# cisco/openh264

Hardware: AMD Instinct MI355X
Metric: 1080p frames/sec/GPU at QP=24 CBP; encoder_binary_comparison SHA1 pass (higher is better)
Workload: dtype u8

## Files before the change

openh264_amd/csrc/kernels/inter_mb.h:

```cpp
#pragma once
#include "frame_kernels.h"
#include "../common/gom_rc.h"


#if defined(WH_EMU)
#include <stdio.h>
static long g_wh_win_stat[40];
static void wh_win_stat_dump() {
  if (!getenv ("WELSHIP_WIN_STATS")) return;
  fprintf (stderr, "welship mb stat: skip %ld bg/static %ld intra %ld p16x16 %ld p16x8 %ld p8x16 %ld p8x8 %ld renamed-skip %ld | searches 16x16 %ld 16x8/8x16 %ld 8x8 %ld, diamond steps %ld %ld %ld | refinements %ld %ld %ld | skip tests %ld with transform %ld\n",
           g_wh_win_stat[8], g_wh_win_stat[9], g_wh_win_stat[10], g_wh_win_stat[11], g_wh_win_stat[12], g_wh_win_stat[13], g_wh_win_stat[14], g_wh_win_stat[15], g_wh_win_stat[16], g_wh_win_stat[17], g_wh_win_stat[18],
           g_wh_win_stat[19], g_wh_win_stat[20], g_wh_win_stat[21], g_wh_win_stat[22], g_wh_win_stat[23], g_wh_win_stat[24], g_wh_win_stat[25], g_wh_win_stat[26]);
  fprintf (stderr, "welship window stat: P macroblocks %ld, reloads %ld, adopted %ld, first loads %ld, mid-walk reloads %ld, chroma predictions inside the window %ld / from the picture %ld\n", g_wh_win_stat[0], g_wh_win_stat[1], g_wh_win_stat[2], g_wh_win_stat[3], g_wh_win_stat[4], g_wh_win_stat[5], g_wh_win_stat[6]);
}
struct WhWinStatInit { WhWinStatInit() { atexit (wh_win_stat_dump); } };
static WhWinStatInit g_wh_win_stat_init;
#define WH_STAT_WIN(i) (++g_wh_win_stat[i])
#define WH_STAT_BLK(base, bw, bh) (++g_wh_win_stat[(base) + ((bw) == 16 && (bh) == 16 ? 0 : (bw) == 8 && (bh) == 8 ? 2 : 1)])
#else
#define WH_STAT_WIN(i) ((void)0)
#define WH_STAT_BLK(base, bw, bh) ((void)0)
#endif

#define WH_REF_NOT_AVAIL (-2)
#define WH_REF_NOT_IN_LIST (-1)
#define WH_WIN_STRIDE 80
#ifndef WH_WIN_ROWS
#define WH_WIN_ROWS 38
#endif
#define WH_WIN_MARGIN_X 19
#ifndef WH_WIN_MARGIN_Y
#define WH_WIN_MARGIN_Y 11
#endif
#ifndef WH_WIN_START
#define WH_WIN_START 5
#endif
#define WH_CWIN_STRIDE 64
#ifndef WH_CWIN_ROWS
#define WH_CWIN_ROWS 24
#endif
#define WH_CWIN_COLS 32

#define WH_SLOT_16x16 0
#define WH_SLOT_8x8 1
#define WH_SLOT_16x8 5
#define WH_SLOT_8x16 7

typedef struct alignas (16) WhWinLds {
  alignas (16) uint8_t win[WH_WIN_ROWS * WH_WIN_STRIDE + 16];
  alignas (16) uint8_t cwin[WH_CWIN_ROWS * WH_CWIN_STRIDE + 16];
} WhWinLds;

typedef struct alignas (16) WhInterLds {
  WhMbLds m;
  uint32_t nb[5 * 36];
  int16_t co_mv[2][2];
  uint32_t sad_cost0_in;
  int16_t mvp_out[16][2];
  int16_t mv_out[16][2];
} WhInterLds;

typedef struct alignas (16) WhInterStage {
  uint32_t cold_pv[64];
} WhInterStage;
typedef struct WhWin { int x0, y0, cx0, cy0; WhWinLds* b; } WhWin;

WH_FN int wh_se_bits (int v) {
// ... 619 lines not shown
#define WH_RF_ACT (lane < nq && (!sub8 || (bw == 16 ? ((lane >> 2) & 3) < 2 : lane < 16)))
#define WH_RF_ENC wh_enc4 (S, ex + (lane < nq ? wh_tl_col (lane, bw) : 0), ey + (lane < nq ? wh_tl_row (lane, bw) : 0))
#define WH_RF_O (wo + (lane < nq ? wh_tl_row (lane, bw) * WH_WIN_STRIDE + wh_tl_col (lane, bw) : 0))
  const int dmx = me.mvx - me.mvpx, dmy = me.mvy - me.mvpy;
  WvLaneArr vG, vhu, vhd, vbl, vbr, vq0, vq1, vq2, vq3;
#if defined(WH_EMU)
  memset (&vG, 0, sizeof (vG)); memset (&vhu, 0, sizeof (vhu)); memset (&vhd, 0, sizeof (vhd)); memset (&vbl, 0, sizeof (vbl)); memset (&vbr, 0, sizeof (vbr));
  memset (&vq0, 0, sizeof (vq0)); memset (&vq1, 0, sizeof (vq1)); memset (&vq2, 0, sizeof (vq2)); memset (&vq3, 0, sizeof (vq3));
#else
  vG = 0; vhu = 0; vhd = 0; vbl = 0; vbr = 0; vq0 = 0; vq1 = 0; vq2 = 0; vq3 = 0;
#endif
  int c_int, c0, c1, c2, c3;
  WV_DECLARE_LANE (lane);
  WV_LANE_EVAL (lane, {
    const int o = WH_RF_O;
    uint32_t a, b;
    WV_LOWN (vG, lane) = (int)wh_ld4u (W.b->win, o);
    wh_rf_h_pair (W.b->win, o, &a, &b); WV_LOWN (vhu, lane) = (int)a; WV_LOWN (vhd, lane) = (int)b;
    wh_rf_b_pair (W.b->win, o, &a, &b); WV_LOWN (vbl, lane) = (int)a; WV_LOWN (vbr, lane) = (int)b; });
  if (satd_in_md) c_int = me.satd_raw;
  else WV_SATD_ROWS_SHARED (c_int, lane, WH_RF_ACT, WH_RF_ENC, (uint32_t)WV_LOWN (vG, lane));
  WV_SATD_ROWS4_SHARED (c0, c1, c2, c3, lane, WH_RF_ACT, WH_RF_ENC, (uint32_t)WV_LOWN (vhu, lane), (uint32_t)WV_LOWN (vhd, lane), (uint32_t)WV_LOWN (vbl, lane), (uint32_t)WV_LOWN (vbr, lane));
  int best = c_int + wh_mvd_cost (C.lambda, dmx, dmy), hb = -1;
  c0 += wh_mvd_cost (C.lambda, dmx, dmy - 2); if (c0 < best) { best = c0; hb = 0; }
  c1 += wh_mvd_cost (C.lambda, dmx, dmy + 2); if (c1 < best) { best = c1; hb = 1; }
  c2 += wh_mvd_cost (C.lambda, dmx - 2, dmy); if (c2 < best) { best = c2; hb = 2; }
  c3 += wh_mvd_cost (C.lambda, dmx + 2, dmy); if (c3 < best) { best = c3; hb = 3; }
  const int hx = hb == 2 ? -2 : hb == 3 ? 2 : 0, hy = hb == 0 ? -2 : hb == 1 ? 2 : 0;
  WV_LANE_EVAL (lane, {
    uint32_t q[4];
    wh_rf_quarters (W.b->win, WH_RF_O, hb, (uint32_t)WV_LOWN (vG, lane), (uint32_t)WV_LOWN (vhu, lane), (uint32_t)WV_LOWN (vhd, lane), (uint32_t)WV_LOWN (vbl, lane), (uint32_t)WV_LOWN (vbr, lane), q);
    WV_LOWN (vq0, lane) = (int)q[0]; WV_LOWN (vq1, lane) = (int)q[1]; WV_LOWN (vq2, lane) = (int)q[2]; WV_LOWN (vq3, lane) = (int)q[3]; });
  WV_SATD_ROWS4_SHARED (c0, c1, c2, c3, lane, WH_RF_ACT, WH_RF_ENC, (uint32_t)WV_LOWN (vq0, lane), (uint32_t)WV_LOWN (vq1, lane), (uint32_t)WV_LOWN (vq2, lane), (uint32_t)WV_LOWN (vq3, lane));
  int qb = -1;
  c0 += wh_mvd_cost (C.lambda, dmx + hx, dmy + hy - 1); if (c0 < best) { best = c0; qb = 0; }
  c1 += wh_mvd_cost (C.lambda, dmx + hx, dmy + hy + 1); if (c1 < best) { best = c1; qb = 1; }
  c2 += wh_mvd_cost (C.lambda, dmx + hx - 1, dmy + hy); if (c2 < best) { best = c2; qb = 2; }
  c3 += wh_mvd_cost (C.lambda, dmx + hx + 1, dmy + hy); if (c3 < best) { best = c3; qb = 3; }
  const int qx = qb == 2 ? -1 : qb == 3 ? 1 : 0, qy = qb == 0 ? -1 : qb == 1 ? 1 : 0;
  me.satd_cost = best;
  WV_LANE_EVAL (lane, {
    if (lane < nq) {
      const int v = qb >= 0 ? (qb == 0 ? WV_LOWN (vq0, lane) : qb == 1 ? WV_LOWN (vq1, lane) : qb == 2 ? WV_LOWN (vq2, lane) : WV_LOWN (vq3, lane))
                  : hb >= 0 ? (hb == 0 ? WV_LOWN (vhu, lane) : hb == 1 ? WV_LOWN (vhd, lane) : hb == 2 ? WV_LOWN (vbl, lane) : WV_LOWN (vbr, lane)) : WV_LOWN (vG, lane);
      * (uint32_t*)&S.m.pred_y[(ey + wh_tl_row (lane, bw)) * 16 + ex + wh_tl_col (lane, bw)] = (uint32_t)v;
    } });
  WV_SYNC();
#undef WH_RF_ACT
#undef WH_RF_ENC
#undef WH_RF_O
  me.mvx += hx + qx; me.mvy += hy + qy;
}

WH_FN int wh_enc_inter_y (WhMbLds& S, int qp) {
  wh_quant_blocks (S, 0, 16, qp, qp, S.res, 0);
  int s0, s1, s2, s3;
  WV_QUADSUM4 (s0, s1, s2, s3, lane, (lane < 16 ? WH_Q_SCORE (S.part2[lane]) : 0));
  int cbp = 0;
  if (s0 + s1 + s2 + s3 >= 6) cbp = (s0 >= 4 ? 1 : 0) | (s1 >= 4 ? 2 : 0) | (s2 >= 4 ? 4 : 0) | (s3 >= 4 ? 8 : 0);
  WV_LANES_BEGIN (lane)
  {
    const int b = lane >> 2, on = (cbp >> (b >> 2)) & 1;
    for (int q = 0; q < 4; ++q) { const int k = (lane & 3) * 4 + q; S.lv_luma[b * 16 + k] = S.res[b * 16 + wh_zigzag (k)]; }
    if (lane < 16) {
      int n = 0;
      if ((cbp >> (lane >> 2)) & 1) n = __builtin_popcount (WH_Q_MASK (S.part2[lane]));
      S.nzc[wh_blk_y (lane) * 4 + wh_blk_x (lane)] = (uint8_t)n;
    }
    (void)on;
  }
  WV_LANES_END
  WV_LANES_BEGIN (lane)
  {
    const int b = lane >> 2, on = (cbp >> (b >> 2)) & 1;
    for (int k = 0; k < 4; ++k) {
      const int i = lane * 4 + k, pos = i & 15;
      S.res[i] = on ? (int16_t) (S.res[i] * wh_dq (qp, pos)) : (int16_t)0;
    }
  }
  WV_LANES_END
  return cbp;
}

WH_FN bool wh_try_py_skip (WhMbLds& S, int qp) {
  wh_quant_blocks (S, 0, 16, qp, qp, S.tmp, 0);
  int bc, u1, u2, u3;
  WV_ROWSUM4 (bc, u1, u2, u3, lane, (lane < 16 ? WH_Q_SCORE (S.part2[lane]) | (WH_Q_BIG (S.part2[lane]) << 16) : 0));
  (void)u1; (void)u2; (void)u3;
  return bc < 6;
}
WH_FN bool wh_try_puv_skip (WhMbLds& S, int qpc) {
  const int ff = wh_ff_inter (qpc, 0) << 1, mf = wh_mf (qpc, 0) >> 1;
  const int16_t thr = (int16_t) (((1 << 16) - 1) / mf - ff);
  for (int pl = 0; pl < 2; ++pl) {
    const int16_t* r = &S.res[256 + pl * 64];
    const int16_t s0 = (int16_t) (r[0] + r[32]), s1 = (int16_t) (r[0] - r[32]), s2 = (int16_t) (r[16] + r[48]), s3 = (int16_t) (r[16] - r[48]);
    const int16_t d0 = (int16_t) (s0 + s2), d1 = (int16_t) (s0 - s2), d2 = (int16_t) (s1 + s3), d3 = (int16_t) (s1 - s3);
    if (wh_abs (d0) > thr || wh_abs (d1) > thr || wh_abs (d2) > thr || wh_abs (d3) > thr) return false;
  }
  wh_quant_blocks (S, 256, 8, qpc, qpc, S.tmp, 1);
  int c0, c1, c2, c3;
  WV_QUADSUM4 (c0, c1, c2, c3, lane, (lane < 8 ? WH_Q_SCORE (S.part2[lane]) | (WH_Q_BIG (S.part2[lane]) << 8) : 0));
  (void)c2; (void)c3;
  return c0 < 7 && c1 < 7;
}

template <int VAR = 0>
WH_FN void wh_inter_cold_fetch (WhInterLds& S, WhInterStage& G, int lane, const WhSeqParams& P, const WhPicJob& J, int mbx, int mby) {
  constexpr bool HOSTIN = VAR == 0 || VAR == 3, CTRL = VAR == 0;
  const int w = P.mb_w, xy = mby * w + mbx;
  wh_ld_async4 ((const WH_G uint8_t*)J.src[0] + WH_SRC_Y_OFF (w, mbx, mby, 0, 0) + lane * 4, (uint32_t*)S.m.enc_y, lane);
  if (lane < 32) wh_ld_async4 ((const WH_G uint8_t*)J.src[0] + WH_SRC_C_OFF (w, mbx, mby, 0, 0, 0) + lane * 4, (uint32_t*)S.m.enc_c, lane);
// ... 120 lines not shown
  }
  const bool bg_cur = bgd && WV_LGET (bgf, 0) != 0, bg_l = bgd && WV_LGET (bgf, 1) != 0, bg_t = bgd && WV_LGET (bgf, 2) != 0;
  const bool bg_tr = bgd && WV_LGET (bgf, 3) != 0, bg_tl = bgd && WV_LGET (bgf, 4) != 0;
  const bool tl_skc = tl_sk && !bg_tl, t_skc = t_sk && !bg_t, tr_skc = tr_sk && !bg_tr, l_skc = l_sk && !bg_l;
  const int sadsk0 = tl_skc ? TLm->skip_sad : 0, sadsk1 = t_skc ? Tm->skip_sad : 0, sadsk2 = tr_skc ? TRm->skip_sad : 0, sadsk3 = l_skc ? Lm->skip_sad : 0;
  const int ref_mb_type = ref_is_p ? Co->mb_type : WH_MB_NONE;
  const bool ref_mb_bg = Co->ref_type == WH_REFTYPE_BACKGROUND;
  WhMeCtx C;
  C.mbx = mbx; C.mby = mby; C.lambda = lambda; C.use_satd = use_satd;
  C.minx = wh_max (- ((mbx + 1) << 4) + 3, -P.mv_range); C.miny = wh_max (- ((mby + 1) << 4) + 3, -P.mv_range);
  C.maxx = wh_min (((P.mb_w - mbx) << 4) - 3, P.mv_range); C.maxy = wh_min (((P.mb_h - mby) << 4) - 3, P.mv_range);

  WH_PROF_MARK (P, M, 10);
  WhMe me16;
  me16.bx = 0; me16.by = 0; me16.bw = 16; me16.bh = 16;
  wh_pred_mv (K, 0, 0, 4, 0, &me16.mvpx, &me16.mvpy);
  WhWin W;
  W.b = X.win;
  WhI16Cost i16c;
  {
    const int icx = wh_clip3 ((2 + me16.mvpx) >> 2, C.minx, C.maxx), icy = wh_clip3 ((2 + me16.mvpy) >> 2, C.miny, C.maxy);
    const int cx = mbx * 16 + icx, cy = mby * 16 + icy;
    const bool adopt = X.spec_valid && wh_win_room (X.spec, cx, cy, 16, 16) >= WH_WIN_START;
    WH_STAT_WIN (0);
    if (adopt) { W.x0 = X.spec.x0; W.y0 = X.spec.y0; W.cx0 = X.spec.cx0; W.cy0 = X.spec.cy0; WH_STAT_WIN (2); WH_PROF_MARK (P, M, 15); }
    else {
      WH_STAT_WIN (3);
      if (X.spec_valid) WV_ASYNC_WAIT();
      wh_win_issue_all (P, J, W, cx, cy);
    }
    wh_i16_costs (M, avail, use_satd, lambda, &i16c);
    WV_ASYNC_WAIT();
  }
  WH_PROF_MARK (P, M, 0);
  int mb_type = WH_MB_P16x16, cbp = 0, cost_luma = 0, cost_skip_mb = 0, sad_cost0 = 0;
  int p16x = 0, p16y = 0;
  int skx = 0, sky = 0;
  bool done = false;

  auto predict_sad_skip = [&] () {
    const int rb = WV_LGET (K.ref, 1), ra = WV_LGET (K.ref, 6);
    int rc = WV_LGET (K.ref, 5);
    const int sb = sadsk1, sa = sadsk3;
    int sc = sadsk2, skip_c = tr_skc;
    if (rc == WH_REF_NOT_AVAIL) { rc = WV_LGET (K.ref, 0); sc = sadsk0; skip_c = tl_skc; }
    if (rb == WH_REF_NOT_AVAIL && rc == WH_REF_NOT_AVAIL && ra != WH_REF_NOT_AVAIL) return sa;
    const int cnt = ((0 == ra) && l_skc) | (((0 == rb) && t_skc) << 1) | (((0 == rc) && skip_c) << 2);
    return cnt == 1 ? sa : cnt == 2 ? sb : cnt == 4 ? sc : wh_median3 (sa, sb, sc);
  };
  const bool try_skip = l_sk || t_sk || tl_sk || tr_sk;
  bool keep_skip = l_sk && t_sk && tr_sk;
  bool b_skip = false;
  const int stale_cbp = ctl.stale_cbp;
  bool bg_coded = false, bg_skip = false, collocated = false;

  if (bgd) {
    keep_skip = keep_skip && !bg_l && !bg_t && !bg_tr;
    const int ref_type_raw = (int)Co->ref_type - 1;
    const bool ref_intra = Co->ref_type != 0 && Co->ref_type != WH_REFTYPE_BACKGROUND && WH_IS_INTRA (ref_type_raw);
    const int ref_qp = Co->ref_qp;
    if (bg_cur && !ref_intra && (ref_qp - qp <= 3  || ref_qp <= 26)) {
      wh_mc_chroma_to (S, P, J, W, mbx, mby, 0, 0, 8, 8, 0, 0, M.pred_c);
      int cb, cr;
      WV_SUM2 (cb, cr, lane, (lane < 16 ? wh_sad4 (* (const uint32_t*)&M.enc_c[lane * 4], * (const uint32_t*)&M.pred_c[lane * 4]) : 0),
               (lane >= 16 && lane < 32 ? wh_sad4 (* (const uint32_t*)&M.enc_c[lane * 4], * (const uint32_t*)&M.pred_c[lane * 4]) : 0));
      const bool too_large = cb > 640 || cr > 640;
      const int chroma_sad = cb + cr, pred_skip = predict_sad_skip();
      const bool cannot = (pred_skip > 128 && chroma_sad >= pred_skip) ||
                          (ref_is_p && ref_mb_type == WH_MB_PSKIP && !ref_mb_bg && Co->skip_sad > 128 && chroma_sad >= Co->skip_sad);
      if (!cannot && !too_large) {
        int sx, sy;
        wh_pred_skip_mv (K, &sx, &sy);
        bg_coded = true; bg_skip = sx == 0 && sy == 0; collocated = true;
        wh_mc_luma_to (S, P, J, W, mbx, mby, 0, 0, 16, 16, 0, 0, M.pred_y);
        const uint8_t* pl = M.pred_y;
        int sad;
        WV_SUM (sad, lane, wh_sad4 (* (const uint32_t*)&M.enc_y[lane * 4], * (const uint32_t*)&pl[lane * 4]));
        sad_cost0 = sad;
        p16x = 0; p16y = 0;
        if (bg_skip) { b_skip = true; mb_type = WH_MB_PSKIP; skx = 0; sky = 0; cost_luma = 0; cost_skip_mb = 0; done = true; }
        else {
          mb_type = WH_MB_P16x16;
          if (md_using_sad) cost_luma = sad;
          else WV_SATD_ROWS (cost_luma, lane, true, wh_enc4 (S, wh_tl_col (lane, 16), wh_tl_row (lane, 16)), * (const uint32_t*)&M.pred_y[wh_tl_row (lane, 16) * 16 + wh_tl_col (lane, 16)]);
          WV_LANES_BEGIN (lane)
          if (lane < 16) { S.mv_out[lane][0] = 0; S.mv_out[lane][1] = 0; S.mvp_out[lane][0] = (int16_t)me16.mvpx; S.mvp_out[lane][1] = (int16_t)me16.mvpy; }
          WV_LANES_END
          wh_dct_luma16 (M);
          cbp = wh_enc_inter_y (M, qp);
          cbp |= wh_encrec_chroma (M, qpc, 0) << 4;
          wh_idct_luma16 (M);
          wh_idct_chroma (M);
          done = true;
        }
      }
    }
  }

  const WH_G WhSccJob* Z = nullptr;
  int idc0 = 0, idc1 = 0, idc2 = 0, idc3 = 0, scroll_on = 0, smx = 0, smy = 0;
  uint32_t dch0 = 0, dch1 = 0, dch2 = 0, dch3 = 0, fme_down_mb = 0;
  bool scd_coded = false;
  if (SCC) {
    Z = (const WH_G WhSccJob*)J.scc;
    const int scd_on = Z->scd_on;
    if (scd_on) {
// ... 23 lines not shown
        const WH_G uint8_t* o0 = (const WH_G uint8_t*)Z->ref_ori_c[0];
        const WH_G uint8_t* o1 = (const WH_G uint8_t*)Z->ref_ori_c[1];
        const ptrdiff_t off = (ptrdiff_t) ((mby << 3) + (oy >> 1)) * P.src_stride_c + (mbx << 3) + (ox >> 1);
        WV_SUM2 (cb, cr, lane,
                 (lane < 16 ? wh_sad4 (* (const uint32_t*)&M.enc_c[lane * 4], wh_ldg4u (o0 + off + (ptrdiff_t) ((lane >> 1) & 7) * P.src_stride_c + (lane & 1) * 4)) : 0),
                 (lane >= 16 && lane < 32 ? wh_sad4 (* (const uint32_t*)&M.enc_c[lane * 4], wh_ldg4u (o1 + off + (ptrdiff_t) ((lane >> 1) & 7) * P.src_stride_c + (lane & 1) * 4)) : 0));
      }
      if (cb != 0 || cr != 0) continue;
      const int ref_qp = Co->ref_qp;
      const bool qp_similar = ref_qp - qp <= 5  || ref_qp <= 26;
      int sx, sy;
      wh_pred_skip_mv (K, &sx, &sy);
      const int vx = (int) (int16_t) (ox * 4), vy = (int) (int16_t) (oy * 4);
      const bool as_skip = qp_similar && sx == vx && sy == vy;
      uint8_t* dy = M.pred_y;
      uint8_t* dc = M.pred_c;
      wh_mc_luma_to (S, P, J, W, mbx, mby, 0, 0, 16, 16, vx, vy, dy);
      wh_mc_chroma_to (S, P, J, W, mbx, mby, 0, 0, 8, 8, vx, vy, dc);
      int sad;
      WV_SUM (sad, lane, wh_sad4 (* (const uint32_t*)&M.enc_y[lane * 4], * (const uint32_t*)&dy[lane * 4]));
      sad_cost0 = sad; cost_skip_mb = sad;
      p16x = vx; p16y = vy;
      scd_coded = true;
      if (as_skip) { b_skip = true; mb_type = WH_MB_PSKIP; skx = vx; sky = vy; cost_luma = 0; collocated = vx == 0 && vy == 0; done = true; WH_STAT (mode ? WH_ST_SCROLL_SKIP : WH_ST_STATIC_SKIP); }
      else {
        WH_STAT (WH_ST_SCD_P16);
        mb_type = WH_MB_P16x16;
        collocated = false;
        if (md_using_sad) cost_luma = sad;
        else cost_luma = wh_cand_sad (S, P, J, W, C, me16, 0, 0);
        WV_LANES_BEGIN (lane)
        if (lane < 16) { S.mv_out[lane][0] = (int16_t)vx; S.mv_out[lane][1] = (int16_t)vy; S.mvp_out[lane][0] = (int16_t)me16.mvpx; S.mvp_out[lane][1] = (int16_t)me16.mvpy; }
        WV_LANES_END
        me16.mvx = vx; me16.mvy = vy;
        wh_dct_luma16 (M);
        cbp = wh_enc_inter_y (M, qp);
        cbp |= wh_encrec_chroma (M, qpc, 0) << 4;
        wh_idct_luma16 (M);
        wh_idct_chroma (M);
        done = true;
      }
    }
  }

  if (!done && ((ref_is_p && ref_mb_type == WH_MB_PSKIP) || try_skip)) {
    const int sad_pred_skip = predict_sad_skip();
    wh_pred_skip_mv (K, &skx, &sky);
    const int nx = (mbx << 4) + (skx >> 2), ny = (mby << 4) + (sky >> 2);
    if (!(nx < -29 || nx > (P.mb_w << 4) + 12 || ny < -29 || ny > (P.mb_h << 4) + 12)) {
      wh_mc_luma_to (S, P, J, W, mbx, mby, 0, 0, 16, 16, skx, sky, M.pred_y);
      WH_PROF_SUB (P, M, 4);
      wh_mc_chroma_to (S, P, J, W, mbx, mby, 0, 0, 8, 8, skx, sky, M.pred_c);
      WH_PROF_SUB (P, M, 5);
      int sad_l, sad_c;
      WV_SUM2 (sad_l, sad_c, lane, wh_sad4 (* (const uint32_t*)&S.m.enc_y[lane * 4], * (const uint32_t*)&M.pred_y[lane * 4]),
               (lane < 32 ? wh_sad4 (* (const uint32_t*)&S.m.enc_c[lane * 4], * (const uint32_t*)&M.pred_c[lane * 4]) : 0));
      const int sad_mb = sad_l + sad_c;
      bool ok = sad_mb == 0 || sad_mb < sad_pred_skip || (ref_is_p && ref_mb_type == WH_MB_PSKIP && !ref_mb_bg && sad_mb < Co->skip_sad);
      WH_PROF_SUB (P, M, 6);
      WH_STAT_WIN (25);
      if (!ok) {
        WH_STAT_WIN (26);
        wh_dct_luma16 (M);
        if (wh_try_py_skip (M, qp)) {
          wh_dct_chroma (M);
          if (wh_try_puv_skip (M, qpc)) ok = true;
        }
      }
      if (ok) {
        b_skip = true;
        if (md_using_sad) cost_luma = sad_l;
        else WV_SATD_ROWS (cost_luma, lane, true, wh_enc4 (S, wh_tl_col (lane, 16), wh_tl_row (lane, 16)), * (const uint32_t*)&M.pred_y[wh_tl_row (lane, 16) * 16 + wh_tl_col (lane, 16)]);
        sad_cost0 = md_using_sad ? sad_l : ((HOSTIN && J.sad_cost0) ? (int)S.sad_cost0_in : Co->sad_cost[0]);
        cost_skip_mb = sad_mb;
        p16x = skx; p16y = sky;
      }
    }
  }
  if (b_skip && keep_skip) { mb_type = WH_MB_PSKIP; done = true; }
  WH_PROF_MARK (P, M, 1);

  int sad_pred16 = 0;
  if (!done && !b_skip && !il_intra) {
    int sad_pred;
    {
      const int rb = WV_LGET (K.ref, 1), ra = WV_LGET (K.ref, 6);
      int rc = WV_LGET (K.ref, 5), sc = sadc2;
      if (rc == WH_REF_NOT_AVAIL) { rc = WV_LGET (K.ref, 0); sc = sadc0; }
      if (rb == WH_REF_NOT_AVAIL && rc == WH_REF_NOT_AVAIL && ra != WH_REF_NOT_AVAIL) sad_pred = sadc3;
      else {
        const int cnt = (0 == ra) | ((0 == rb) << 1) | ((0 == rc) << 2);
        sad_pred = cnt == 1 ? sadc3 : cnt == 2 ? sadc1 : cnt == 4 ? sc : wh_median3 (sadc3, sadc1, sc);
      }
      const int v = sad_pred << 6;
      sad_pred = ((v - (v >> 3) + (v >> 5)) + 32) >> 6;
    }
    int nm = 1;
    const bool c_l = Lm != nullptr, c_t = Tm != nullptr, c_r = ref_is_p && mbx < P.mb_w - 1, c_b = ref_is_p && mby < P.mb_h - 1;
    const int i_l = 1, i_t = i_l + (c_l ? 1 : 0), i_r = i_t + (c_t ? 1 : 0), i_b = i_r + (c_r ? 1 : 0);
    nm = i_b + (c_b ? 1 : 0);
    WV_LSET (mvcl, 0, il_mv);
    if (c_l) WV_LSET (mvcl, i_l, wh_pk_mv (Lm->p16mv[0], Lm->p16mv[1]));
    if (c_t) WV_LSET (mvcl, i_t, wh_pk_mv (Tm->p16mv[0], Tm->p16mv[1]));
    const int msh = HOSTIN ? J.mvc_shift : 0;
    if (c_r) WV_LSET (mvcl, i_r, wh_pk_mv (S.co_mv[0][0] >> msh, S.co_mv[0][1] >> msh));
    if (c_b) WV_LSET (mvcl, i_b, wh_pk_mv (S.co_mv[1][0] >> msh, S.co_mv[1][1] >> msh));
    me16.sad_pred = sad_pred;
    if (SCC) {
      WhSccMe z;
      z.job = Z; z.method = 1; z.thr = Z->thr16; z.dir_on = 0; z.dmx = 0; z.dmy = 0; z.chain = 0; z.fme_down = 0;
      wh_motion_search (S, P, J, W, C, me16, mvcl, nm, &z);
    } else wh_motion_search (S, P, J, W, C, me16, mvcl, nm);
    p16x = me16.mvx; p16y = me16.mvy;
    cost_luma = me16.satd_cost;
    mb_type = WH_MB_P16x16;
    sad_pred16 = sad_pred;
  }

// ... 106 lines not shown
      else if (sign == 6 || sign == 9) order0 = 0;
      else if (sign != 15) { order0 = 0; order1 = 1; order2 = 2; chain = true; }
    } else {
      order0 = 0; order1 = 1; order2 = 2; chain = true;
    }
    int best_cost = cost_luma;
    for (int oi = 0; oi < 3; ++oi) {
      const int g = oi == 0 ? order0 : oi == 1 ? order1 : order2;
      if (g < 0) break;
      const int first = g == 0 ? WH_SLOT_8x8 : g == 1 ? WH_SLOT_16x8 : WH_SLOT_8x16, cnt = g == 0 ? 4 : 2;
      int c = 0;
      for (int i = 0; i < cnt; ++i) {
        WhMe m;
        wh_slot_geom (first + i, &m.bx, &m.by, &m.bw, &m.bh);
        m.sad_pred = g == 0 ? sad_pred16 >> 2 : sad_pred16 >> 1;
        wh_slot_pred (K, first + i, &m.mvpx, &m.mvpy);
        wh_motion_search (S, P, J, W, C, m, mvcl, 1);
        wh_cache_set (K, m.bx >> 2, m.by >> 2, m.bw >> 2, m.bh >> 2, 0, m.mvx, m.mvy);
        wh_me_store (T, first + i, m);
        c += m.satd_cost;
      }
      if (oi == 0) {
        if (c < best_cost) { best_cost = c; mb_type = g == 0 ? WH_MB_P8x8 : g == 1 ? WH_MB_P16x8 : WH_MB_P8x16; }
        else if (chain) break;
      } else if (c <= best_cost) { best_cost = c; mb_type = g == 1 ? WH_MB_P16x8 : WH_MB_P8x16; }
    }

    WH_PROF_MARK (P, M, 4);
    const int satd_in_md = use_satd;
    int best_sad = 0, best_satd = 0;
    if (mb_type == WH_MB_P8x8) {
      WV_LSET (K.ref, 9, WH_REF_NOT_AVAIL); WV_LSET (K.ref, 21, WH_REF_NOT_AVAIL);
    }
    {
      const int first = mb_type == WH_MB_P16x16 ? WH_SLOT_16x16 : mb_type == WH_MB_P16x8 ? WH_SLOT_16x8 : mb_type == WH_MB_P8x16 ? WH_SLOT_8x16 : WH_SLOT_8x8;
      const int cnt = mb_type == WH_MB_P16x16 ? 1 : mb_type == WH_MB_P8x8 ? 4 : 2;
      for (int i = 0; i < cnt; ++i) {
        WhMe m;
        wh_slot_geom (first + i, &m.bx, &m.by, &m.bw, &m.bh);
        wh_me_fetch (T, first + i, m);
        wh_slot_pred (K, first + i, &m.mvpx, &m.mvpy);
        wh_refine_frac (S, P, J, W, C, m, satd_in_md, merged ? 1 : 0);
        wh_cache_set (K, m.bx >> 2, m.by >> 2, m.bw >> 2, m.bh >> 2, 0, m.mvx, m.mvy);
        {
          const int bx4 = m.bx >> 2, by4 = m.by >> 2, w4 = m.bw >> 2, h4 = m.bh >> 2;
          WV_LANES_BEGIN (lane)
          if (lane < w4 * h4) {
            const int r = (by4 + (w4 == 4 ? lane >> 2 : lane >> 1)) * 4 + bx4 + (lane & (w4 - 1));
            S.mv_out[r][0] = (int16_t)m.mvx; S.mv_out[r][1] = (int16_t)m.mvy; S.mvp_out[r][0] = (int16_t)m.mvpx; S.mvp_out[r][1] = (int16_t)m.mvpy;
          }
          WV_LANES_END
        }
        best_sad += m.sad_cost; best_satd += m.satd_cost;
        wh_mc_chroma_to (S, P, J, W, mbx, mby, m.bx >> 1, m.by >> 1, m.bw >> 1, m.bh >> 1, m.mvx, m.mvy, M.pred_c);
        if (mb_type == WH_MB_P16x16) { me16.mvx = m.mvx; me16.mvy = m.mvy; }
      }
    }
    if (mb_type == WH_MB_P16x16) {
      int sl, sc;
      WV_SUM2 (sl, sc, lane, wh_sad4 (* (const uint32_t*)&M.enc_y[lane * 4], * (const uint32_t*)&M.pred_y[lane * 4]),
               (lane < 32 ? wh_sad4 (* (const uint32_t*)&M.enc_c[lane * 4], * (const uint32_t*)&M.pred_c[lane * 4]) : 0));
      cost_skip_mb = sl + sc;
    }
    sad_cost0 = best_sad;
    cost_luma = md_using_sad ? best_sad : best_satd;

    WH_PROF_MARK (P, M, 5);
    publish_guess (wh_pk_mv (p16x, p16y));
  }
  if (searched) {
    wh_dct_luma16 (M);
    cbp = wh_enc_inter_y (M, qp);
    const int cbp_c = wh_encrec_chroma (M, qpc, 0);
    cbp |= cbp_c << 4;
    wh_idct_luma16 (M);
    wh_idct_chroma (M);
    if (mb_type == WH_MB_P16x16 && cbp == 0) {
      int sx, sy;
      wh_pred_skip_mv (K, &sx, &sy);
      if (sx == me16.mvx && sy == me16.mvy) { mb_type = WH_MB_PSKIP; skx = sx; sky = sy; }
    }
  }

  WH_PROF_MARK (P, M, 6);
  const bool is_skip = mb_type == WH_MB_PSKIP;
  WH_STAT_WIN (intra ? 10 : (bg_coded || scd_coded) ? 9 : (is_skip && b_skip) ? 8 : is_skip ? 15 : mb_type == WH_MB_P16x16 ? 11 : mb_type == WH_MB_P16x8 ? 12 : mb_type == WH_MB_P8x16 ? 13 : 14);
  WH_G WhMbState* Ms = (WH_G WhMbState*)J.mbs + xy;
  WH_G WhMbRecord* Rs = (WH_G WhMbRecord*)J.records + xy;
  if (intra) {
    WV_LANES_BEGIN (lane)
    if (lane < 16) { wh_st_x<XWG> ((WH_G uint32_t*)&Ms->mv[lane][0], 0u); Rs->mvd[lane][0] = 0; Rs->mvd[lane][1] = 0; }
    if (lane < 2) Rs->mv_tr[lane] = 0;
    if (lane < 4) { wh_st_x<XWG> (&Ms->ref_idx[lane], (int8_t)-1); Rs->ref_idx[lane] = -1; Rs->sub_type[lane] = 0; }
    if (lane == 0) { wh_st_x<XWG> (&Ms->sad_cost[0], 0); wh_st_x<XWG> ((WH_G uint32_t*)&Ms->p16mv[0], (uint32_t)wh_pk_mv (p16x, p16y)); wh_st_x<XWG> (&Ms->skip_sad, 0); if (HOSTIN && J.sad_cost0) (J.sad_cost0_out ? (WH_G int32_t*)J.sad_cost0_out : (WH_G int32_t*)J.sad_cost0)[xy] = 0; }
    WV_LANES_END
    int ibits = 0;
    if (CTRL && J.want_bits) {
      ibits = wh_mb_residual_bits (M, ir.mb_type, ir.cbp, Lm ? Lm->nzc : nullptr, Tm ? Tm->nzc : nullptr) +
              wh_mb_intra_header_bits (M, ir.mb_type, ir.cbp, ir.i16_mode_std, ir.chroma_mode_std, true);
      if (ir.cbp > 0 || ir.mb_type == WH_MB_I16x16) ibits |= WH_BITS_HAS_QP_DELTA;
    }
    wh_store_mb<XWG> (M, P, J, mbx, mby, ir.mb_type, ir.cbp, qp, qpc, ir.i16_mode_std, ir.chroma_mode_std, ir.cost_luma, slice_idc, ibits);
    if (SCC && J.dyn_slice) {
      WV_LANES_BEGIN (lane)
      if (lane == 0) Rs->fme_down = 0;
      WV_LANES_END
    }
    return;
  }
  if (is_skip && b_skip) {
    WV_LANES_BEGIN (lane)
    {
      const int row = lane >> 2, seg = lane & 3;
      * (uint32_t*)&WH_RY (M, seg * 4, row) = * (const uint32_t*)&M.pred_y[row * 16 + seg * 4];
    }
    if (lane < 32) {
      const int pl = lane >> 4, row = (lane >> 1) & 7, half = lane & 1;
      * (uint32_t*)&WH_RC (M, pl, half * 4, row) = * (const uint32_t*)&M.pred_c[pl * 64 + row * 8 + half * 4];
    }
    if (lane < 24) M.nzc[lane] = 0;
    WV_LANES_END
    cbp = 0;
  }
  WV_LANES_BEGIN (lane)
  if (lane < 16) {
    const int mvx = is_skip ? skx : S.mv_out[lane][0], mvy = is_skip ? sky : S.mv_out[lane][1];
    const uint32_t mv32 = (uint32_t)wh_pk_mv (mvx, mvy);
    wh_st_x<XWG> ((WH_G uint32_t*)&Ms->mv[lane][0], mv32);
    * (WH_G uint32_t*)&Rs->mvd[lane][0] = is_skip ? 0u : (uint32_t)wh_pk_mv (mvx - S.mvp_out[lane][0], mvy - S.mvp_out[lane][1]);
// ... 79 lines not shown
```

openh264_amd/csrc/kernels/mb_common.h:

```cpp
#pragma once
#include "prims.h"

typedef struct WhMbLds {
  uint8_t  enc_y[256];
  uint8_t  enc_c[128];
  uint8_t  rec_y[17 * 32];
  uint8_t  rec_c[2][9 * 16];
  uint8_t  pred_y[256];
  uint8_t  pred_c[128];
  uint8_t  pred4[9 * 16];
  int16_t  res[384];
  int16_t  tmp[256];
  int32_t  part[64];
  int32_t  part2[16];
  int16_t  dc[16];
  int16_t  cdc[8];
  int8_t   i4m[25];
  uint8_t  nzc[24];
  alignas (8) int16_t lv_luma[256];
  int16_t  lv_dc[16];
  alignas (8) int16_t lv_cac[128];
  int16_t  lv_cdc[8];
  int8_t   i4_rem[16];
  uint16_t i4_prev;
// ... 64 lines not shown
  WV_LANES_END
}

WH_FN void wh_idct_luma16 (WhMbLds& S) {
  WV_LANES_BEGIN (lane)
  const int b = lane >> 2, r = lane & 3;
  const int16_t* c = &S.res[b * 16 + r * 4];
  int16_t t0, t1, t2, t3;
  wh_idct4_h (c[0], c[1], c[2], c[3], &t0, &t1, &t2, &t3);
  int16_t* t = &S.tmp[b * 16 + r * 4];
  t[0] = t0; t[1] = t1; t[2] = t2; t[3] = t3;
  WV_LANES_END
  WV_LANES_BEGIN (lane)
  const int b = lane >> 2, c = lane & 3;
  const int16_t* t = &S.tmp[b * 16 + c];
  int r0, r1, r2, r3;
  wh_idct4_v (t[0], t[4], t[8], t[12], &r0, &r1, &r2, &r3);
  const int px = wh_blk_x (b) * 4 + c, py = wh_blk_y (b) * 4;
  WH_RY (S, px, py + 0) = wh_clip255 (S.pred_y[(py + 0) * 16 + px] + r0);
  WH_RY (S, px, py + 1) = wh_clip255 (S.pred_y[(py + 1) * 16 + px] + r1);
  WH_RY (S, px, py + 2) = wh_clip255 (S.pred_y[(py + 2) * 16 + px] + r2);
  WH_RY (S, px, py + 3) = wh_clip255 (S.pred_y[(py + 3) * 16 + px] + r3);
  WV_LANES_END
}

WH_FN void wh_idct_chroma (WhMbLds& S) {
  WV_LANES_BEGIN (lane)
  if (lane < 32) {
    const int b = lane >> 2, r = lane & 3;
    const int16_t* c = &S.res[256 + b * 16 + r * 4];
    int16_t t0, t1, t2, t3;
    wh_idct4_h (c[0], c[1], c[2], c[3], &t0, &t1, &t2, &t3);
    int16_t* t = &S.tmp[b * 16 + r * 4];
    t[0] = t0; t[1] = t1; t[2] = t2; t[3] = t3;
  }
  WV_LANES_END
  WV_LANES_BEGIN (lane)
  if (lane < 32) {
    const int b = lane >> 2, c = lane & 3;
    const int pl = b >> 2, bb = b & 3;
    const int16_t* t = &S.tmp[b * 16 + c];
    int r0, r1, r2, r3;
    wh_idct4_v (t[0], t[4], t[8], t[12], &r0, &r1, &r2, &r3);
    const int px = (bb & 1) * 4 + c, py = (bb >> 1) * 4;
    const uint8_t* p = &S.pred_c[pl * 64];
    WH_RC (S, pl, px, py + 0) = wh_clip255 (p[(py + 0) * 8 + px] + r0);
    WH_RC (S, pl, px, py + 1) = wh_clip255 (p[(py + 1) * 8 + px] + r1);
    WH_RC (S, pl, px, py + 2) = wh_clip255 (p[(py + 2) * 8 + px] + r2);
    WH_RC (S, pl, px, py + 3) = wh_clip255 (p[(py + 3) * 8 + px] + r3);
  }
  WV_LANES_END
}

WH_FN int wh_cost_luma16 (WhMbLds& S, int use_satd) {
  int cost;
  if (!use_satd) {
    WV_SUM (cost, lane, (wh_abs (S.enc_y[lane * 4 + 0] - S.pred_y[lane * 4 + 0]) + wh_abs (S.enc_y[lane * 4 + 1] - S.pred_y[lane * 4 + 1]) +
                          wh_abs (S.enc_y[lane * 4 + 2] - S.pred_y[lane * 4 + 2]) + wh_abs (S.enc_y[lane * 4 + 3] - S.pred_y[lane * 4 + 3])));
    return cost;
  }
  WV_LANES_BEGIN (lane)
  const int b = lane >> 2, r = lane & 3;
  const int px = (b & 3) * 4, py = (b >> 2) * 4 + r;
  const uint8_t* e = &S.enc_y[py * 16 + px];
  const uint8_t* p = &S.pred_y[py * 16 + px];
  int o0, o1, o2, o3;
  wh_had4 (e[0] - p[0], e[1] - p[1], e[2] - p[2], e[3] - p[3], &o0, &o1, &o2, &o3);
  int16_t* t = &S.tmp[b * 16 + r * 4];
  t[0] = (int16_t)o0; t[1] = (int16_t)o1; t[2] = (int16_t)o2; t[3] = (int16_t)o3;
  WV_LANES_END
  WV_LANES_BEGIN (lane)
  const int b = lane >> 2, c = lane & 3;
  const int16_t* t = &S.tmp[b * 16 + c];
  int o0, o1, o2, o3;
  wh_had4 (t[0], t[4], t[8], t[12], &o0, &o1, &o2, &o3);
  S.part[lane] = wh_abs (o0) + wh_abs (o1) + wh_abs (o2) + wh_abs (o3);
  WV_LANES_END
  WV_SUM (cost, lane, (lane < 16 ? ((S.part[lane * 4] + S.part[lane * 4 + 1] + S.part[lane * 4 + 2] + S.part[lane * 4 + 3] + 1) >> 1) : 0));
  return cost;
}

WH_FN int wh_cost_chroma (WhMbLds& S, int use_satd) {
  int cost;
  if (!use_satd) {
    WV_SUM (cost, lane, (lane < 32 ? (wh_abs (S.enc_c[lane * 4 + 0] - S.pred_c[lane * 4 + 0]) + wh_abs (S.enc_c[lane * 4 + 1] - S.pred_c[lane * 4 + 1]) +
                                        wh_abs (S.enc_c[lane * 4 + 2] - S.pred_c[lane * 4 + 2]) + wh_abs (S.enc_c[lane * 4 + 3] - S.pred_c[lane * 4 + 3])) : 0));
    return cost;
  }
  WV_LANES_BEGIN (lane)
  if (lane < 32) {
    const int b = lane >> 2, r = lane & 3;
    const int pl = b >> 2, bb = b & 3;
    const int px = (bb & 1) * 4, py = (bb >> 1) * 4 + r;
    const uint8_t* e = &S.enc_c[pl * 64 + py * 8 + px];
    const uint8_t* p = &S.pred_c[pl * 64 + py * 8 + px];
    int o0, o1, o2, o3;
    wh_had4 (e[0] - p[0], e[1] - p[1], e[2] - p[2], e[3] - p[3], &o0, &o1, &o2, &o3);
    int16_t* t = &S.tmp[b * 16 + r * 4];
    t[0] = (int16_t)o0; t[1] = (int16_t)o1; t[2] = (int16_t)o2; t[3] = (int16_t)o3;
  }
  WV_LANES_END
  WV_LANES_BEGIN (lane)
  if (lane < 32) {
    const int b = lane >> 2, c = lane & 3;
    const int16_t* t = &S.tmp[b * 16 + c];
    int o0, o1, o2, o3;
// ... 254 lines not shown
      if (ll < 4 && (h ? nz1 : nz0) > 0) {
        const int16_t* t = &S.tmp[h * 16 + ll];
        int r0, r1, r2, r3;
        wh_idct4_v (t[0], t[4], t[8], t[12], &r0, &r1, &r2, &r3);
        const uint8_t* p = &pr[slot * 16 + ll];
        WH_RY (S, bx + ll, by + 0) = wh_clip255 (p[0] + r0);
        WH_RY (S, bx + ll, by + 1) = wh_clip255 (p[4] + r1);
        WH_RY (S, bx + ll, by + 2) = wh_clip255 (p[8] + r2);
        WH_RY (S, bx + ll, by + 3) = wh_clip255 (p[12] + r3);
      }
    }
    WV_LANES_END
  }
#undef WH_I4P_HALF
}

WH_FN int wh_single_ctr_mask (unsigned m) {
  const unsigned R = m << 6, M = R | 63u;
  const unsigned a1 = M << 1, a3 = a1 | (M << 2) | (M << 3), a6 = a3 | (M << 4) | (M << 5) | (M << 6);
  return __builtin_popcount (R & a1) + __builtin_popcount (R & a3) + __builtin_popcount (R & a6);
}
#define WH_Q_MASK(w) ((unsigned)(w) & 0xffffu)
#define WH_Q_SCORE(w) ((int)(((unsigned)(w) >> 16) & 0xffu))
#define WH_Q_BIG(w) ((int)(((unsigned)(w) >> 24) & 1u))
#define WH_Q_ANY(w) ((int)(((unsigned)(w) >> 25) & 1u))
WH_FN void wh_quant_blocks (WhMbLds& S, int base, int nblk, int qp, int ffrow, int16_t* dst, int skip_dc) {
  WV_LANES_BEGIN (lane)
  if (lane < nblk * 4) {
    int16_t mx = 0;
    unsigned pm = 0;
    const unsigned inv4 = (unsigned) (0xFEA9DB83C7426510ULL >> (16 * (lane & 3))) & 0xffffu;
    for (int k = 0; k < 4; ++k) {
      const int i = lane * 4 + k, pos = i & 15;
      int16_t a;
      dst[i] = wh_quant1_abs_t (S.res[base + i], wh_ff_row (ffrow, pos), wh_mf (qp, pos), &a);
      if (mx < a) mx = a;
      pm |= (unsigned) (a != 0) << ((inv4 >> (4 * k)) & 15u);
    }
    S.part[lane] = (int32_t) (pm | ((unsigned) (uint16_t)mx << 16));
  }
  WV_LANES_END
  WV_LANES_BEGIN (lane)
  if (lane < nblk) {
    const unsigned w0 = (unsigned)S.part[lane * 4], w1 = (unsigned)S.part[lane * 4 + 1], w2 = (unsigned)S.part[lane * 4 + 2], w3 = (unsigned)S.part[lane * 4 + 3];
    const unsigned m = ((w0 | w1 | w2 | w3) & 0xffffu) >> skip_dc;
    const int mx = wh_max (wh_max ((int) (w0 >> 16), (int) (w1 >> 16)), wh_max ((int) (w2 >> 16), (int) (w3 >> 16)));
    const unsigned big = mx > 1, any = mx != 0;
    const unsigned score = big ? 9u : (unsigned)wh_single_ctr_mask (m);
    S.part2[lane] = (int32_t) (m | (score << 16) | (big << 24) | (any << 25));
  }
  WV_LANES_END
}

WH_FN int wh_encrec_chroma (WhMbLds& S, int qpc, int is_intra) {
  wh_dct_chroma (S);
  const int ffrow = is_intra ? qpc + 6 : qpc;
  WV_LANES_BEGIN (lane)
  if (lane < 2) {
    int16_t* r = &S.res[256 + lane * 64];
    const int16_t s0 = (int16_t) (r[0] + r[32]), s1 = (int16_t) (r[0] - r[32]);
    const int16_t s2 = (int16_t) (r[16] + r[48]), s3 = (int16_t) (r[16] - r[48]);
    r[0] = 0; r[16] = 0; r[32] = 0; r[48] = 0;
    const int ff = kWhQuantFF[ffrow * 3 + 0] << 1, mf = kWhQuantMF[qpc * 3 + 0] >> 1;
    int16_t* d = &S.cdc[lane * 4];
    d[0] = wh_quant1_t ((int16_t) (s0 + s2), ff, mf);
    d[1] = wh_quant1_t ((int16_t) (s0 - s2), ff, mf);
    d[2] = wh_quant1_t ((int16_t) (s1 + s3), ff, mf);
    d[3] = wh_quant1_t ((int16_t) (s1 - s3), ff, mf);
    for (int k = 0; k < 4; ++k) S.lv_cdc[lane * 4 + k] = d[k];
  }
  WV_LANES_END
  wh_quant_blocks (S, 256, 8, qpc, ffrow, &S.res[256], 1);
  int sc0, sc1, nzdc0, nzdc1;
#define WH_CSCORE(l) (is_intra ? (WH_Q_ANY (S.part2[l]) ? 7 : 0) : WH_Q_SCORE (S.part2[l]))
  WV_QUADSUM4 (sc0, sc1, nzdc0, nzdc1, lane, (lane < 8 ? WH_CSCORE (lane & 7) : lane < 16 ? (int) (S.cdc[lane & 7] != 0) : 0));
#undef WH_CSCORE
  const int keep0 = sc0 >= 7, keep1 = sc1 >= 7;
  WV_LANES_BEGIN (lane)
  {
    if (lane < 32) {
      const int b = lane >> 2;
      for (int q = 0; q < 4; ++q) {
        const int k = (lane & 3) * 4 + q;
        S.lv_cac[b * 16 + k] = (k < 15) ? S.res[256 + b * 16 + wh_zigzag (k + 1)] : (int16_t)0;
      }
    }
    if (lane < 8) {
      int n = 0;
      if (lane < 4 ? keep0 : keep1) n = __builtin_popcount (WH_Q_MASK (S.part2[lane]));
      S.nzc[16 + lane] = (uint8_t)n;
    }
  }
  WV_LANES_END
  WV_LANES_BEGIN (lane)
  for (int h = 0; h < 2; ++h) {
    const int i = lane + 64 * h, keep = h == 0 ? keep0 : keep1;
    S.res[256 + i] = keep ? (int16_t) (S.res[256 + i] * wh_dq (qpc, i & 15)) : (int16_t)0;
  }
  WV_LANES_END
  if (nzdc0 > 0 || nzdc1 > 0) {
    WV_LANES_BEGIN (lane)
    if (lane < 2 && (lane == 0 ? nzdc0 : nzdc1) > 0) {
      int16_t* d = &S.cdc[lane * 4];
      const int16_t su = (int16_t) (d[0] + d[2]), du = (int16_t) (d[0] - d[2]);
      const int16_t sd = (int16_t) (d[1] + d[3]), dd = (int16_t) (d[1] - d[3]);
      const int mf = wh_dq (qpc, 0);
      int16_t* r = &S.res[256 + lane * 64];
      r[0]  = (int16_t) (((su + sd) * mf) >> 1);
      r[16] = (int16_t) (((su - sd) * mf) >> 1);
      r[32] = (int16_t) (((du + dd) * mf) >> 1);
      r[48] = (int16_t) (((du - dd) * mf) >> 1);
    }
    WV_LANES_END
  }
  return (keep0 || keep1) ? 2 : (nzdc0 > 0 || nzdc1 > 0) ? 1 : 0;
}
```

Measured before the change: 27540.

## Reuse P_Skip test chroma prediction and transforms, skip IDCT for zero-CBP blocks

When the P_Skip test already computed the chroma prediction and the luma/chroma DCTs, and the searched 16x16 vector matches the skip vector, those results are reused rather than recomputed. Luma and chroma encoding gain a lean early-exit when the CBP is zero, and reconstruction then copies the prediction instead of running dequant and IDCT. This removes redundant motion compensation, transform and inverse-transform work per macroblock. It adds state-tracking complexity, and bit-exactness depends on the reused buffers not having been overwritten in between. Stat counters are added under the emulator build.

```diff
diff --git a/openh264_amd/csrc/kernels/inter_mb.h b/openh264_amd/csrc/kernels/inter_mb.h
--- a/openh264_amd/csrc/kernels/inter_mb.h
+++ b/openh264_amd/csrc/kernels/inter_mb.h
@@ -11,8 +11,11 @@
   fprintf (stderr, "welship mb stat: skip %ld bg/static %ld intra %ld p16x16 %ld p16x8 %ld p8x16 %ld p8x8 %ld renamed-skip %ld | searches 16x16 %ld 16x8/8x16 %ld 8x8 %ld, diamond steps %ld %ld %ld | refinements %ld %ld %ld | skip tests %ld with transform %ld\n",
            g_wh_win_stat[8], g_wh_win_stat[9], g_wh_win_stat[10], g_wh_win_stat[11], g_wh_win_stat[12], g_wh_win_stat[13], g_wh_win_stat[14], g_wh_win_stat[15], g_wh_win_stat[16], g_wh_win_stat[17], g_wh_win_stat[18],
            g_wh_win_stat[19], g_wh_win_stat[20], g_wh_win_stat[21], g_wh_win_stat[22], g_wh_win_stat[23], g_wh_win_stat[24], g_wh_win_stat[25], g_wh_win_stat[26]);
+  fprintf (stderr, "welship skip-reuse stat: searched %ld, with something left by the P_Skip test %ld (dropped: vector differs %ld, other partition shape %ld) | reused: chroma prediction %ld luma transform %ld chroma transform %ld | reconstruction copied: luma cbp 0 %ld chroma cbp 0 %ld\n",
+           g_wh_win_stat[32], g_wh_win_stat[33], g_wh_win_stat[34], g_wh_win_stat[35], g_wh_win_stat[27], g_wh_win_stat[28], g_wh_win_stat[29], g_wh_win_stat[30], g_wh_win_stat[31]);
   fprintf (stderr, "welship window stat: P macroblocks %ld, reloads %ld, adopted %ld, first loads %ld, mid-walk reloads %ld, chroma predictions inside the window %ld / from the picture %ld\n", g_wh_win_stat[0], g_wh_win_stat[1], g_wh_win_stat[2], g_wh_win_stat[3], g_wh_win_stat[4], g_wh_win_stat[5], g_wh_win_stat[6]);
 }
+extern "C" __attribute__ ((visibility ("default"))) long WelsEmuMbStat (int i) { return i >= 0 && i < 40 ? g_wh_win_stat[i] : -1; }
 struct WhWinStatInit { WhWinStatInit() { atexit (wh_win_stat_dump); } };
 static WhWinStatInit g_wh_win_stat_init;
 #define WH_STAT_WIN(i) (++g_wh_win_stat[i])
@@ -738,12 +741,18 @@
   me.mvx += hx + qx; me.mvy += hy + qy;
 }
 
-WH_FN int wh_enc_inter_y (WhMbLds& S, int qp) {
+WH_FN int wh_enc_inter_y (WhMbLds& S, int qp, bool lean = false) {
   wh_quant_blocks (S, 0, 16, qp, qp, S.res, 0);
   int s0, s1, s2, s3;
   WV_QUADSUM4 (s0, s1, s2, s3, lane, (lane < 16 ? WH_Q_SCORE (S.part2[lane]) : 0));
   int cbp = 0;
   if (s0 + s1 + s2 + s3 >= 6) cbp = (s0 >= 4 ? 1 : 0) | (s1 >= 4 ? 2 : 0) | (s2 >= 4 ? 4 : 0) | (s3 >= 4 ? 8 : 0);
+  if (lean && cbp == 0) {
+    WV_LANES_BEGIN (lane)
+    if (lane < 16) S.nzc[lane] = 0;
+    WV_LANES_END
+    return 0;
+  }
   WV_LANES_BEGIN (lane)
   {
     const int b = lane >> 2, on = (cbp >> (b >> 2)) & 1;
@@ -970,6 +979,8 @@
   bool keep_skip = l_sk && t_sk && tr_sk;
   bool b_skip = false;
   const int stale_cbp = ctl.stale_cbp;
+  enum { WH_SKL_PRED_C = 1, WH_SKL_DCT_Y = 2, WH_SKL_DCT_C = 4 };
+  int skip_left = 0, sk_sad_mb = 0;
   bool bg_coded = false, bg_skip = false, collocated = false;
 
   if (bgd) {
@@ -1099,18 +1110,23 @@
       WH_PROF_SUB (P, M, 4);
       wh_mc_chroma_to (S, P, J, W, mbx, mby, 0, 0, 8, 8, skx, sky, M.pred_c);
       WH_PROF_SUB (P, M, 5);
+      const bool track = !SCC && !bgd && !il_intra;
+      if (track) skip_left = WH_SKL_PRED_C;
       int sad_l, sad_c;
       WV_SUM2 (sad_l, sad_c, lane, wh_sad4 (* (const uint32_t*)&S.m.enc_y[lane * 4], * (const uint32_t*)&M.pred_y[lane * 4]),
                (lane < 32 ? wh_sad4 (* (const uint32_t*)&S.m.enc_c[lane * 4], * (const uint32_t*)&M.pred_c[lane * 4]) : 0));
       const int sad_mb = sad_l + sad_c;
+      sk_sad_mb = sad_mb;
       bool ok = sad_mb == 0 || sad_mb < sad_pred_skip || (ref_is_p && ref_mb_type == WH_MB_PSKIP && !ref_mb_bg && sad_mb < Co->skip_sad);
       WH_PROF_SUB (P, M, 6);
       WH_STAT_WIN (25);
       if (!ok) {
         WH_STAT_WIN (26);
         wh_dct_luma16 (M);
+        if (track) skip_left |= WH_SKL_DCT_Y;
         if (wh_try_py_skip (M, qp)) {
           wh_dct_chroma (M);
+          if (track) skip_left |= WH_SKL_DCT_C;
           if (wh_try_puv_skip (M, qpc)) ok = true;
         }
       }
@@ -1323,11 +1339,18 @@
           WV_LANES_END
         }
         best_sad += m.sad_cost; best_satd += m.satd_cost;
-        wh_mc_chroma_to (S, P, J, W, mbx, mby, m.bx >> 1, m.by >> 1, m.bw >> 1, m.bh >> 1, m.mvx, m.mvy, M.pred_c);
+        if (skip_left) {
+          WH_STAT_WIN (33);
+          if (mb_type != WH_MB_P16x16) { skip_left = 0; WH_STAT_WIN (35); }
+          else if (m.mvx != skx || m.mvy != sky) { skip_left = 0; WH_STAT_WIN (34); }
+        }
+        if (skip_left & WH_SKL_PRED_C) WH_STAT_WIN (27);
+        else wh_mc_chroma_to (S, P, J, W, mbx, mby, m.bx >> 1, m.by >> 1, m.bw >> 1, m.bh >> 1, m.mvx, m.mvy, M.pred_c);
         if (mb_type == WH_MB_P16x16) { me16.mvx = m.mvx; me16.mvy = m.mvy; }
       }
     }
-    if (mb_type == WH_MB_P16x16) {
+    if (mb_type == WH_MB_P16x16 && (skip_left & WH_SKL_PRED_C)) cost_skip_mb = sk_sad_mb;
+    else if (mb_type == WH_MB_P16x16) {
       int sl, sc;
       WV_SUM2 (sl, sc, lane, wh_sad4 (* (const uint32_t*)&M.enc_y[lane * 4], * (const uint32_t*)&M.pred_y[lane * 4]),
                (lane < 32 ? wh_sad4 (* (const uint32_t*)&M.enc_c[lane * 4], * (const uint32_t*)&M.pred_c[lane * 4]) : 0));
@@ -1340,12 +1363,19 @@
     publish_guess (wh_pk_mv (p16x, p16y));
   }
   if (searched) {
-    wh_dct_luma16 (M);
-    cbp = wh_enc_inter_y (M, qp);
-    const int cbp_c = wh_encrec_chroma (M, qpc, 0);
+    WH_STAT_WIN (32);
+    if (skip_left & WH_SKL_DCT_Y) WH_STAT_WIN (28);
+    else wh_dct_luma16 (M);
+    cbp = wh_enc_inter_y (M, qp, true);
+    if (skip_left & WH_SKL_DCT_C) WH_STAT_WIN (29);
+    const int cbp_c = wh_encrec_chroma (M, qpc, 0, (skip_left & WH_SKL_DCT_C) != 0, true);
+    const bool zero_y = cbp == 0, zero_c = cbp_c == 0;
+    if (zero_y) WH_STAT_WIN (30);
+    if (zero_c) WH_STAT_WIN (31);
     cbp |= cbp_c << 4;
-    wh_idct_luma16 (M);
-    wh_idct_chroma (M);
+    if (!zero_y) wh_idct_luma16 (M);
+    if (!zero_c) wh_idct_chroma (M);
+    if (zero_y || zero_c) wh_rec_copy_pred (M, zero_y, zero_c);
     if (mb_type == WH_MB_P16x16 && cbp == 0) {
       int sx, sy;
       wh_pred_skip_mv (K, &sx, &sy);
diff --git a/openh264_amd/csrc/kernels/mb_common.h b/openh264_amd/csrc/kernels/mb_common.h
--- a/openh264_amd/csrc/kernels/mb_common.h
+++ b/openh264_amd/csrc/kernels/mb_common.h
@@ -140,6 +140,19 @@
   WV_LANES_END
 }
 
+WH_FN void wh_rec_copy_pred (WhMbLds& S, bool luma, bool chroma) {
+  WV_LANES_BEGIN (lane)
+  if (luma) {
+    const int row = lane >> 2, seg = lane & 3;
+    * (uint32_t*)&WH_RY (S, seg * 4, row) = * (const uint32_t*)&S.pred_y[row * 16 + seg * 4];
+  }
+  if (chroma && lane < 32) {
+    const int pl = lane >> 4, row = (lane >> 1) & 7, half = lane & 1;
+    * (uint32_t*)&WH_RC (S, pl, half * 4, row) = * (const uint32_t*)&S.pred_c[pl * 64 + row * 8 + half * 4];
+  }
+  WV_LANES_END
+}
+
 WH_FN int wh_cost_luma16 (WhMbLds& S, int use_satd) {
   int cost;
   if (!use_satd) {
@@ -500,8 +513,8 @@
   WV_LANES_END
 }
 
-WH_FN int wh_encrec_chroma (WhMbLds& S, int qpc, int is_intra) {
-  wh_dct_chroma (S);
+WH_FN int wh_encrec_chroma (WhMbLds& S, int qpc, int is_intra, bool have_dct = false, bool lean = false) {
+  if (!have_dct) wh_dct_chroma (S);
   const int ffrow = is_intra ? qpc + 6 : qpc;
   WV_LANES_BEGIN (lane)
   if (lane < 2) {
@@ -540,6 +553,7 @@
     }
   }
   WV_LANES_END
+  if (lean && !keep0 && !keep1 && nzdc0 == 0 && nzdc1 == 0) return 0;
   WV_LANES_BEGIN (lane)
   for (int h = 0; h < 2; ++h) {
     const int i = lane + 64 * h, keep = h == 0 ? keep0 : keep1;
```

After: 27770 (median of 6 runs). No clear change (+0.9%).
